# sarvex/redpanda

Measured on AMD Instinct MI355X. Metric: record-batch validate+parse(+decompress) GB/s per GPU and per 8-GPU node, higher is better.
Workload: dtype u8; 1 GPU; C2: 1,048,576 uncompressed Kafka v2 batches x 16,381 B (16 records x (16 B key + 995 B value)), 4096 partitions per GPU; Kafka CRC32C + internal header CRC + record walk + offset/timestamp index; batches_per_gpu=1048576, batches_total=1048576, partitions_total=4096, partitions_per_gpu=4096, parallelism=partition-shard x1

## Files before the change

### redpanda_amd/_build.py

```python
from __future__ import annotations

import os
import subprocess
from pathlib import Path

PKG = Path(__file__).resolve().parent
ROOT = PKG.parent
CSRC = PKG / "csrc"
INCLUDE = ROOT / "include"
CONDA = Path(os.environ.get("RPGPU_CODEC_PREFIX", "/opt/conda"))
ARCH = os.environ.get("PYTORCH_ROCM_ARCH", "gfx950")

LIBRPGPU = PKG / "librpgpu.so"
LIBRPGEN = PKG / "librpgen.so"

RPGPU_SRCS = ["rpgpu_kernels.hip", "rpgpu_decomp.hip", "rpgpu_sets.hip", "rpgpu_index.hip", "rpgpu_summary.hip", "rpgpu_compact.hip", "rpgpu_compact_rw.hip", "rpgpu_fetch.hip", "rpgpu_compress.hip", "rpgpu_stamp.hip", "rpgpu_legacy.hip", "rpgpu_pp.hip", "rpgpu_abi.cpp", "rpgpu_tables.cpp"]
RPGPU_HDRS = ["rpgpu_internal.h", "rpgpu_device.h", "rpgpu_walk.h", "rpgpu_copy.h", "rpgpu_legacy.h", "rpgpu_pp.h", "rpgpu_codec.h", "rpgpu_zstd.h", "rpgpu_zseq.h", "rpgpu_zblk.h", "rpgpu_wave.h", "rpgpu_inflate.h", "rpgpu_lz4c.h", "rpgpu_snappyc.h", "rpgpu_deflatec.h", "rpgpu_zstdc.h"]
RPGEN_SRCS = ["rpgen.cpp"]
RPGEN_HDRS = ["rpgen.h"]


def _stale(out: Path, srcs: list[Path]) -> bool:
    if not out.exists():
        return True
    t = out.stat().st_mtime
    return any(s.stat().st_mtime > t for s in srcs)


def _run(cmd: list[str]) -> None:
    r = subprocess.run(cmd, capture_output=True, text=True)
    if r.returncode != 0:
        raise RuntimeError(f"build failed: {' '.join(cmd)}\n{r.stdout}\n{r.stderr}")


def build_rpgpu(force: bool = False) -> Path:
    srcs = [CSRC / s for s in RPGPU_SRCS + RPGPU_HDRS] + [INCLUDE / "rpgpu.h"]
    if force or _stale(LIBRPGPU, srcs):
        from concurrent.futures import ThreadPoolExecutor

        obj = ROOT / "build" / "obj"
        obj.mkdir(parents=True, exist_ok=True)
        flags = [f"--offload-arch={ARCH}", "-O3", "-std=c++17", "-fPIC", f"-I{INCLUDE}", f"-I{CSRC}"]
        objs = [obj / (s + ".o") for s in RPGPU_SRCS]
        jobs = max(1, min(len(objs), os.cpu_count() or 1, 8))
        with ThreadPoolExecutor(jobs) as ex:
            list(ex.map(lambda so: _run(["hipcc", *flags, "-c", str(CSRC / so[0]), "-o", str(so[1])]),
                        zip(RPGPU_SRCS, objs)))
        tmp = LIBRPGPU.with_suffix(".so.tmp")
        _run(["hipcc", f"--offload-arch={ARCH}", "-shared", *[str(o) for o in objs], "-o", str(tmp)])
        os.replace(tmp, LIBRPGPU)
    return LIBRPGPU


def build_rpgen(force: bool = False) -> Path:
    srcs = [CSRC / s for s in RPGEN_SRCS + RPGEN_HDRS] + [INCLUDE / "rpgpu.h"]
    if force or _stale(LIBRPGEN, srcs):
        tmp = LIBRPGEN.with_suffix(".so.tmp")
        _run(["g++", "-O3", "-std=c++17", "-fPIC", "-shared", "-pthread",
              f"-I{INCLUDE}", f"-I{CSRC}", f"-I{CONDA / 'include'}",
              *[str(CSRC / s) for s in RPGEN_SRCS],
              f"-L{CONDA / 'lib'}", f"-Wl,-rpath,{CONDA / 'lib'}",
              "-llz4", "-lzstd", "-lsnappy", "-lz", "-o", str(tmp)])
        os.replace(tmp, LIBRPGEN)
    return LIBRPGEN


def build_all(force: bool = False) -> None:
    build_rpgpu(force)
    build_rpgen(force)


if __name__ == "__main__":
    build_all(force=True)
    print("built", LIBRPGPU, LIBRPGEN)
```

### redpanda_amd/csrc/rpgpu_kernels.hip

```cpp
#include "rpgpu_device.h"
#include "rpgpu_walk.h"

namespace rpgpu {

#ifdef RPGPU_DIAG_STAMPS
__device__ unsigned long long g_stamps[8];
struct Stamps {
    uint64_t st[8];
    uint64_t prev;
};
#define DIAG_PARAM , Stamps& sp
#define DIAG_PASS , sp
#define STAMP(i)                                          \
    do {                                                  \
        const uint64_t _t = __builtin_amdgcn_s_memtime(); \
        sp.st[i] += _t - sp.prev;                         \
        sp.prev = _t;                                     \
    } while (0)
#else
#define DIAG_PARAM
#define DIAG_PASS
#define STAMP(i) \
    do {         \
    } while (0)
#endif

struct Header {
    int32_t size_bytes;
    int64_t base_offset;
    int32_t type;
    int32_t crc;
    int16_t attrs;
    int32_t last_offset_delta;
    int64_t first_ts, max_ts, producer_id;
    int16_t producer_epoch;
    int32_t base_sequence, record_count;
};

struct Result {
    int32_t verdict;
    uint32_t crc, crc_expected, header_crc;
    Header h;
    uint32_t index_first, index_count;
};

__device__ __forceinline__ uint32_t u32s(uint32_t v) { return (uint32_t)__builtin_amdgcn_readfirstlane((int)v); }
__device__ __forceinline__ void write_result(rpgpu_batch_result* out, const Result& r) {
    if (lane_id() == 0) {
        const uint64_t bo = (uint64_t)r.h.base_offset, ft = (uint64_t)r.h.first_ts, mt = (uint64_t)r.h.max_ts;
        u32x4 a = {u32s((uint32_t)r.verdict), u32s(r.crc), u32s(r.crc_expected), u32s(r.header_crc)};
        u32x4 b = {u32s((uint32_t)r.h.size_bytes), u32s((uint32_t)r.h.record_count), u32s((uint32_t)bo),
                   u32s((uint32_t)(bo >> 32))};
        u32x4 c = {u32s((uint32_t)r.h.last_offset_delta),
                   u32s((uint32_t)(uint16_t)r.h.attrs | ((uint32_t)(r.h.attrs & 7) << 16) |
                        ((uint32_t)(uint8_t)r.h.type << 24)),
                   u32s((uint32_t)ft), u32s((uint32_t)(ft >> 32))};
        u32x4 d = {u32s((uint32_t)mt), u32s((uint32_t)(mt >> 32)), u32s(r.index_first), u32s(r.index_count)};
        u32x4* o = reinterpret_cast<u32x4*>(out);
        o[0] = a;
        o[1] = b;
        o[2] = c;
        o[3] = d;
    }
}

__device__ __forceinline__ void load_tables(uint32_t* s, const uint32_t* __restrict__ g) {
    for (int i = threadIdx.x; i < kTableWords / 4; i += blockDim.x)
        reinterpret_cast<u32x4*>(s)[i] = reinterpret_cast<const u32x4*>(g)[i];
    __syncthreads();
}

__device__ __forceinline__ uint32_t header_crc_vec(const uint32_t* sT, const Img64& D) {
    uint32_t win[16];
    win[0] = 0;
    win[1] = (D.w[1] << 24) ^ 0xff000000u;
    win[2] = ((D.w[1] >> 8) | (D.w[2] << 24)) ^ 0x00ffffffu;
#pragma unroll
    for (int m = 3; m < 16; m++) win[m] = (D.w[m - 1] >> 8) | (D.w[m] << 24);
    const uint32_t l = lane_id();
    uint32_t vwin = 0;
#pragma unroll
    for (int i = 0; i < 16; i++) vwin = writelane(vwin, win[i], i);
    const uint32_t w = __builtin_amdgcn_ds_bpermute((int)((l >> 2) << 2), vwin);
    const uint32_t byte = (w >> (8 * (l & 3))) & 255u;
    const uint32_t* hb = sT + kOffHB + l;
    uint32_t c = hb[(byte & 15u) * 64] ^ hb[(16u + (byte >> 4)) * 64];
    c ^= row_shl<1>(c);
    c ^= row_shl<2>(c);
    c ^= row_shl<4>(c);
    c ^= row_shl<8>(c);
    return ~(rdl(c, 0) ^ rdl(c, 16) ^ rdl(c, 32) ^ rdl(c, 48));
}

struct Geom {
    int32_t niter, g0;
};
__device__ __forceinline__ Geom geometry(int32_t n) {
    const int32_t niter = (n - 21 + 1023) >> 10;
    return Geom{niter, n - (niter << 10)};
}
__device__ __forceinline__ int32_t chunk_rows(int32_t niter) {
    return (niter + kRowsPerChunk - 1) & ~(kRowsPerChunk - 1);
}

struct Prefetch {
    u32x4 x[kRowsPerChunk];
    uint32_t hv;
    Geom gm;
};

typedef int32_t i32x4 __attribute__((ext_vector_type(4)));
__device__ __forceinline__ __amdgpu_buffer_rsrc_t batch_rsrc(const uint8_t* p) {
    return __builtin_amdgcn_make_buffer_rsrc(const_cast<uint8_t*>(p), 0, 0x7ffffff0, 0x00020000);
}
#ifndef RPGPU_ROW_AUX
#define RPGPU_ROW_AUX 2
#endif
__device__ __forceinline__ u32x4 load_row(__amdgpu_buffer_rsrc_t rs, const Geom& gm, int32_t row, uint32_t l) {
    const int32_t rb = row < gm.niter ? gm.g0 + (row << 10) : (int32_t)0x80000000;
    const i32x4 v = __builtin_amdgcn_raw_buffer_load_b128(rs, rb + (int32_t)(16 * l), 0, RPGPU_ROW_AUX);
    return (u32x4){(uint32_t)v.x, (uint32_t)v.y, (uint32_t)v.z, (uint32_t)v.w};
}

__device__ __forceinline__ void load_rows(u32x4 (&x)[kRowsPerChunk], __amdgpu_buffer_rsrc_t rs, const Geom& gm,
                                          int32_t cb, uint32_t l) {
#pragma unroll
    for (int k = 0; k < kRowsPerChunk; k++) x[k] = load_row(rs, gm, cb + k, l);
}

__device__ __forceinline__ Geom desc_geometry(const rpgpu_batch_desc& d) {
    return (d.length >= (uint32_t)kHeaderSize && !(d.flags & RPGPU_DESC_NULL_RECORDS)) ? geometry((int32_t)d.length)
                                                                                      : Geom{0, 0};
}

__device__ __forceinline__ u32x4 merge_header(u32x4 y, int32_t ro0, uint32_t v_img, uint32_t l) {
    if (ro0 >= kHeaderSize) return y;
    const int32_t ro = ro0 + 16 * (int32_t)l;
#pragma unroll
    for (int q = 0; q < 4; q++) {
        const int32_t o4 = ro + 4 * q;
        const uint32_t im = img_dword(v_img, o4);
        uint32_t keep;
        if (o4 >= kHeaderSize)
            keep = 0xffffffffu;
        else if (o4 + 4 <= kHeaderSize)
            keep = 0;
        else
            keep = 0xffffffffu << (8 * (uint32_t)(kHeaderSize - o4));
        const uint32_t raw = q == 0 ? y.x : q == 1 ? y.y : q == 2 ? y.z : y.w;
        const uint32_t v = (raw & keep) | (o4 >= kHeaderSize ? 0u : im);
        if (q == 0) y.x = v;
        if (q == 1) y.y = v;
        if (q == 2) y.z = v;
        if (q == 3) y.w = v;
    }
    return y;
}

__device__ __forceinline__ void process_batch(const uint32_t* __restrict__ sT, const rpgpu_batch_desc& d,
                                              uint32_t b, const uint8_t* __restrict__ data,
                                              rpgpu_batch_result* __restrict__ res, uint32_t index_first,
                                              Prefetch& pf, const rpgpu_batch_desc& nd,
                                              bool has_next DIAG_PARAM) {
    const uint32_t l = lane_id();
    const uint8_t* p = data + d.offset;
    const uint32_t len = d.length;
    Result r;
    r.verdict = RPGPU_V_OK;
    r.crc = r.crc_expected = r.header_crc = 0;
    r.h.size_bytes = r.h.type = r.h.crc = r.h.last_offset_delta = 0;
    r.h.base_sequence = r.h.record_count = 0;
    r.h.attrs = r.h.producer_epoch = 0;
    r.h.base_offset = r.h.first_ts = r.h.max_ts = r.h.producer_id = 0;
    r.index_first = index_first;
    r.index_count = 0;

    const uint32_t hv = pf.hv;
    Img64 H;
#pragma unroll
    for (int i = 0; i < 16; i++) H.w[i] = rdl(hv, i);
    Geom ngm{0, 0};
    const __amdgpu_buffer_rsrc_t nrs = batch_rsrc(data + (has_next ? nd.offset : 0));
    pf.hv = (uint32_t)__builtin_amdgcn_raw_buffer_load_b32(nrs, (int32_t)(4 * (l & 15)), 0, 0);
    if (has_next) ngm = desc_geometry(nd);

    Img64 D;
    D.clear();
    int64_t n;
    bool body_trunc = false;
    bool fail = false;
    if (d.flags & RPGPU_DESC_NULL_RECORDS) {
        n = 0;
        r.verdict = RPGPU_V_NULL_RECORDS;
        fail = true;
    } else if (d.format == RPGPU_FMT_KAFKA_WIRE) {
        const int32_t bl = (int32_t)H.get_be(8, 4);
        const uint64_t blen = (uint64_t)(int64_t)bl + 12u;
        if (blen <= (uint64_t)len) {
            n = (int64_t)blen;
        } else {
            n = len;
            body_trunc = true;
        }
        if (len < 12) {
            r.verdict = RPGPU_V_TOO_SMALL;
            fail = true;
        } else if (n < 17) {
            r.verdict = RPGPU_V_HDR_TRUNC_THROW;
            fail = true;
        } else if ((int8_t)H.byte(16) != 2) {
            r.verdict = RPGPU_V_BAD_MAGIC;
            fail = true;
        } else if (n < kHeaderSize) {
            r.verdict = RPGPU_V_HDR_TRUNC_THROW;
            fail = true;
        } else {
            r.h.size_bytes = (int32_t)((uint32_t)bl + 12u);
            r.h.base_offset = (int64_t)H.get_be(0, 8);
            r.h.type = 1;
            r.h.crc = (int32_t)H.get_be(17, 4);
            r.h.attrs = (int16_t)H.get_be(21, 2);
            r.h.last_offset_delta = (int32_t)H.get_be(23, 4);
            r.h.first_ts = (int64_t)H.get_be(27, 8);
            r.h.max_ts = (int64_t)H.get_be(35, 8);
            r.h.producer_id = (int64_t)H.get_be(43, 8);
            r.h.producer_epoch = (int16_t)H.get_be(51, 2);
            r.h.base_sequence = (int32_t)H.get_be(53, 4);
            r.h.record_count = (int32_t)H.get_be(57, 4);
            D.put_le(4, (uint32_t)r.h.size_bytes, 4);
            D.put_le(8, (uint64_t)r.h.base_offset, 8);
            D.put_le(16, 1, 1);
            D.put_le(17, (uint32_t)r.h.crc, 4);
            D.put_le(21, (uint16_t)r.h.attrs, 2);
            D.put_le(23, (uint32_t)r.h.last_offset_delta, 4);
            D.put_le(27, (uint64_t)r.h.first_ts, 8);
            D.put_le(35, (uint64_t)r.h.max_ts, 8);
            D.put_le(43, (uint64_t)r.h.producer_id, 8);
            D.put_le(51, (uint16_t)r.h.producer_epoch, 2);
            D.put_le(53, (uint32_t)r.h.base_sequence, 4);
            D.put_le(57, (uint32_t)r.h.record_count, 4);
        }
    } else {
        n = 0;
        if (len < kHeaderSize) {
            r.verdict = RPGPU_V_STREAM_SHORT;
            fail = true;
        } else {
            uint32_t any = 0;
#pragma unroll
            for (int i = 0; i < 15; i++) any |= H.w[i];
            any |= H.w[15] & 0xffu;
            if (any == 0) {
                r.verdict = RPGPU_V_FALLOCATED_ZERO;
                fail = true;
            } else {
#pragma unroll
                for (int i = 0; i < 16; i++) D.w[i] = H.w[i];
                D.w[15] &= 0xffu;
                r.h.size_bytes = (int32_t)H.get_le(4, 4);
                r.h.base_offset = (int64_t)H.get_le(8, 8);
                r.h.type = (int8_t)H.byte(16);
                r.h.crc = (int32_t)H.get_le(17, 4);
                r.h.attrs = (int16_t)H.get_le(21, 2);
                r.h.last_offset_delta = (int32_t)H.get_le(23, 4);
                r.h.first_ts = (int64_t)H.get_le(27, 8);
                r.h.max_ts = (int64_t)H.get_le(35, 8);
                r.h.producer_id = (int64_t)H.get_le(43, 8);
                r.h.producer_epoch = (int16_t)H.get_le(51, 2);
                r.h.base_sequence = (int32_t)H.get_le(53, 4);
                r.h.record_count = (int32_t)H.get_le(57, 4);
                n = (int64_t)r.h.size_bytes;
            }
        }
    }
    const bool is_disk = d.format != RPGPU_FMT_KAFKA_WIRE;
    const bool recrc = is_disk && (d.ops & RPGPU_OP_RECRC);
    if (!fail) {
        r.crc_expected = (uint32_t)r.h.crc;
        if (!recrc && ((d.ops & RPGPU_OP_HDRCRC) || is_disk)) r.header_crc = header_crc_vec(sT, D);
        if (is_disk) {
            if (!recrc && r.header_crc != H.w[0]) {
                r.verdict = RPGPU_V_HDR_CRC_MISMATCH;
                fail = true;
            } else if (r.h.size_bytes < kHeaderSize || (int64_t)r.h.size_bytes > (int64_t)len) {
                r.verdict = RPGPU_V_STREAM_SHORT;
                fail = true;
            }
        }
    }
    if (fail) {
        load_rows(pf.x, nrs, ngm, 0, l);
        pf.gm = ngm;
        write_result(res + b, r);
        return;
    }

    Img64 B;
    B.clear();
    B.put_be(21, (uint16_t)r.h.attrs, 2);
    B.put_be(23, (uint32_t)r.h.last_offset_delta, 4);
    B.put_be(27, (uint64_t)r.h.first_ts, 8);
    B.put_be(35, (uint64_t)r.h.max_ts, 8);
    B.put_be(43, (uint64_t)r.h.producer_id, 8);
    B.put_be(51, (uint16_t)r.h.producer_epoch, 2);
    B.put_be(53, (uint32_t)r.h.base_sequence, 4);
    B.put_be(57, (uint32_t)r.h.record_count, 4);
    B.w[5] ^= 0xffffff00u;
    B.w[6] ^= 0x000000ffu;
    uint32_t v_img = 0;
#pragma unroll
    for (int i = 0; i < 16; i++) v_img = (l == (uint32_t)i) ? B.w[i] : v_img;

    const Geom gm = geometry((int32_t)n);
    const int32_t nrows = chunk_rows(gm.niter);
    const bool pf_ok = pf.gm.niter == gm.niter && pf.gm.g0 == gm.g0;
    const uint32_t* sN = sT + kOffN;
    const __amdgpu_buffer_rsrc_t rs = batch_rsrc(p);
    const __amdgpu_buffer_rsrc_t nrs_rows = batch_rsrc(data + (has_next ? nd.offset : 0));
    uint32_t c = 0;
    STAMP(0);
    if (!pf_ok) load_rows(pf.x, rs, gm, 0, l);
    pf.x[0] = merge_header(pf.x[0], gm.g0, v_img, l);
    pf.x[1] = merge_header(pf.x[1], gm.g0 + 1024, v_img, l);
    for (int32_t cb = 0; cb < nrows; cb += kRowsPerChunk) {
        const bool last_chunk = cb + kRowsPerChunk >= nrows;
        const __amdgpu_buffer_rsrc_t lrs = last_chunk ? nrs_rows : rs;
        const Geom lg = last_chunk ? ngm : gm;
        const int32_t lrow = last_chunk ? 0 : cb + kRowsPerChunk;
#pragma unroll
        for (int k = 0; k < kRowsPerChunk; k++) {
            u32x4 y = pf.x[k];
            y.x ^= c;
            c = crc_block(sN, y);
            pf.x[k] = load_row(lrs, lg, lrow + k, l);
        }
    }
    pf.gm = ngm;
    STAMP(1);
#ifndef RPGPU_DIAG_NO_COMBINE
    c = combine64(sT + kOffW, c);
    if (nrows != gm.niter) c = apply8(sT + kOffU + (nrows - gm.niter) * 128, c);
#endif
    r.crc = ~rdl(c, 0);
#if defined(RPGPU_DIAG_NO_COMBINE) || defined(RPGPU_DIAG_NO_LOOKUP)
    asm volatile("" ::"v"(c));
    r.crc = r.crc_expected;
#endif
    if (recrc) {
        r.crc_expected = r.crc;
        r.h.crc = (int32_t)r.crc;
        D.put_le(17, r.crc, 4);
        r.header_crc = header_crc_vec(sT, D);
    }
    STAMP(2);

    const uint8_t codec = (uint8_t)(r.h.attrs & 7);
    if (r.crc != r.crc_expected) {
        r.verdict = RPGPU_V_CRC_MISMATCH;
    } else if (body_trunc) {
        r.verdict = RPGPU_V_BODY_TRUNC_THROW;
    } else if (codec > 4) {
        r.verdict = RPGPU_V_BAD_CODEC_THROW;
    }
    write_result(res + b, r);
    STAMP(3);
}

__global__ __launch_bounds__(kValidateThreads) void validate_kernel(
    const rpgpu_batch_desc* __restrict__ descs, uint32_t b0, uint32_t n, const uint8_t* __restrict__ data,
    rpgpu_batch_result* __restrict__ res, rpgpu_record_index* __restrict__ index,
    const uint32_t* __restrict__ local_first, const uint32_t* __restrict__ caps,
    const uint64_t* __restrict__ block_base, uint64_t index_cap, const uint32_t* __restrict__ tables) {
    __shared__ __attribute__((aligned(16))) uint32_t sT[kTableWords];
    load_tables(sT, tables);
    const uint32_t wave = threadIdx.x >> 6;
    const uint32_t gw = __builtin_amdgcn_readfirstlane(blockIdx.x * kWavesPerBlock + wave);
    const uint32_t nw = gridDim.x * kWavesPerBlock;
#ifdef RPGPU_DIAG_STAMPS
    Stamps sp{};
    sp.prev = __builtin_amdgcn_s_memtime();
#endif
    Prefetch pf;
    pf.gm = Geom{0, 0};
    if (b0 + gw < n) {
        const rpgpu_batch_desc d0 = sload_desc(descs + b0 + gw);
        const uint8_t* p0 = data + d0.offset;
        const __amdgpu_buffer_rsrc_t rs0 = batch_rsrc(p0);
        pf.hv = (uint32_t)__builtin_amdgcn_raw_buffer_load_b32(rs0, (int32_t)(4 * (lane_id() & 15)), 0, 0);
        pf.gm = desc_geometry(d0);
        load_rows(pf.x, rs0, pf.gm, 0, lane_id());
    }
    for (uint32_t b = b0 + gw; b < n; b += nw) {
        const rpgpu_batch_desc d = sload_desc(descs + b);
        const bool has_next = b + nw < n;
        const rpgpu_batch_desc nd = sload_desc(descs + (has_next ? b + nw : b));
        process_batch(sT, d, b, data, res, 0u, pf, nd, has_next DIAG_PASS);
        STAMP(5);
    }
#ifdef RPGPU_DIAG_STAMPS
    if (lane_id() == 0)
        for (int i = 0; i < 6; i++) atomicAdd(&g_stamps[i], (unsigned long long)sp.st[i]);
#endif
}

__global__ __launch_bounds__(256) void walk_kernel(const rpgpu_batch_desc* __restrict__ descs, uint32_t b0,
                                                   uint32_t n,
                                                   const uint8_t* __restrict__ data,
                                                   rpgpu_batch_result* __restrict__ res,
                                                   rpgpu_record_index* __restrict__ index,
                                                   const uint32_t* __restrict__ local_first,
                                                   const uint32_t* __restrict__ caps,
                                                   const uint64_t* __restrict__ block_base, uint64_t index_cap,
                                                   uint32_t* __restrict__ wave_list, uint32_t* __restrict__ wave_count) {
    const uint32_t b = b0 + blockIdx.x * blockDim.x + threadIdx.x;
    WalkJob J;
    J.flags = 0;
    J.body = 0;
    J.base_offset = J.first_ts = 0;
    J.n = J.first = J.cap = J.b = 0;
    J.rc = 0;
    uint32_t first_all = 0;
    if (b < n) {
        const rpgpu_batch_desc d = descs[b];
        const rpgpu_batch_result& r = res[b];
        const uint64_t first = block_base[b / kScanBlock] + local_first[b];
        first_all = (uint32_t)first;
        if ((d.ops & (RPGPU_OP_PARSE | RPGPU_OP_INDEX)) && r.verdict == RPGPU_V_OK && r.codec == 0) {
            uint64_t cap = caps[b];
            if (first >= index_cap) cap = 0;
            else if (first + cap > index_cap) cap = index_cap - first;
            J.body = d.offset + kHeaderSize;
            J.base_offset = r.base_offset;
            J.first_ts = r.first_timestamp;
            J.n = (uint32_t)r.size_bytes - kHeaderSize;
            J.rc = r.record_count;
            J.first = (uint32_t)first;
            J.cap = (uint32_t)cap;
            J.b = b;
            J.flags = kJobLive | ((d.ops & RPGPU_OP_INDEX) ? kJobIndex : 0u);
            if (J.rc > kWaveWalkMin) {
                wave_list[atomicAdd(wave_count, 1u)] = b;
                J.flags = 0;
            }
        }
    }
    walk_lanes(data, J, index, res);
    if (b < n && !(J.flags & kJobLive)) reinterpret_cast<uint32_t*>(res + b)[14] = first_all;
}

__global__ __launch_bounds__(256) void walk_wave_kernel(const rpgpu_batch_desc* __restrict__ descs,
                                                        const uint8_t* __restrict__ data,
                                                        rpgpu_batch_result* __restrict__ res,
                                                        rpgpu_record_index* __restrict__ index,
                                                        const uint32_t* __restrict__ local_first,
                                                        const uint32_t* __restrict__ caps,
                                                        const uint64_t* __restrict__ block_base, uint64_t index_cap,
                                                        const uint32_t* __restrict__ wave_list,
                                                        const uint32_t* __restrict__ wave_count,
                                                        uint32_t* __restrict__ head) {
    const uint32_t cnt = *wave_count;
    for (;;) {
        uint32_t k = 0;
        if (lane_id() == 0) k = atomicAdd(head, 1u);
        k = __builtin_amdgcn_readfirstlane(k);
        if (k >= cnt) break;
        const uint32_t b = wave_list[k];
        const rpgpu_batch_desc d = descs[b];
        const rpgpu_batch_result& r = res[b];
        const uint64_t first = block_base[b / kScanBlock] + local_first[b];
        uint64_t cap = caps[b];
        if (first >= index_cap) cap = 0;
        else if (first + cap > index_cap) cap = index_cap - first;
        WalkJob J;
        J.body = d.offset + kHeaderSize;
        J.base_offset = r.base_offset;
        J.first_ts = r.first_timestamp;
        J.n = (uint32_t)r.size_bytes - kHeaderSize;
        J.rc = r.record_count;
        J.first = (uint32_t)first;
        J.cap = (uint32_t)cap;
        J.b = b;
        J.flags = kJobLive | ((d.ops & RPGPU_OP_INDEX) ? kJobIndex : 0u);
        int32_t verdict;
        uint32_t count;
        wave_walk_batch(data, J, index, verdict, count);
        if (lane_id() == 0) {
            uint32_t* o = reinterpret_cast<uint32_t*>(res + b);
            o[0] = (uint32_t)verdict;
            o[15] = count;
        }
    }
}

__device__ __forceinline__ uint32_t index_cap(const rpgpu_batch_desc& d, const uint8_t* data) {
    if (!(d.ops & (RPGPU_OP_PARSE | RPGPU_OP_INDEX)) || (d.flags & RPGPU_DESC_NULL_RECORDS)) return 0;
    const uint8_t* p = data + d.offset;
    const uint64_t len = d.length;
    if (len < (uint64_t)kHeaderSize) return 0;
    uint64_t n;
    int32_t rc;
    uint32_t attrs;
    if (d.format == RPGPU_FMT_KAFKA_WIRE) {
        const int32_t bl = (int32_t)bswap32(ld4(p + 8));
        const uint64_t blen = (uint64_t)(int64_t)bl + 12u;
        if (blen > len) return 0;
        n = blen;
        if (n < (uint64_t)kHeaderSize || p[16] != 2) return 0;
        attrs = ((uint32_t)p[21] << 8) | p[22];
        rc = (int32_t)bswap32(ld4(p + 57));
    } else {
        const int32_t sz = (int32_t)ld4(p + 4);
        if (sz < kHeaderSize || (uint64_t)sz > len) return 0;
        n = (uint64_t)sz;
        attrs = ((uint32_t)p[22] << 8) | p[21];
        rc = (int32_t)ld4(p + 57);
    }
    if ((attrs & 7u) != 0 || rc <= 0) return 0;
    uint64_t cap = (n - kHeaderSize) / 2;
    if ((uint64_t)rc < cap) cap = (uint64_t)rc;
    return (uint32_t)cap;
}

__global__ __launch_bounds__(kScanBlock) void caps_kernel(const rpgpu_batch_desc* __restrict__ descs,
                                                          uint32_t n, const uint8_t* __restrict__ data,
                                                          uint32_t* __restrict__ caps,
                                                          uint32_t* __restrict__ local_first,
                                                          uint64_t* __restrict__ block_sum) {
    __shared__ uint32_t wsum[kScanBlock / 64];
    const uint32_t i = blockIdx.x * kScanBlock + threadIdx.x;
    uint32_t cap = 0;
    if (i < n) cap = index_cap(descs[i], data);
    const uint32_t l = lane_id();
    uint32_t x = cap;
#pragma unroll
    for (int s = 1; s < 64; s <<= 1) {
        uint32_t t = __shfl_up(x, s, 64);
        if (l >= (uint32_t)s) x += t;
    }
    const uint32_t wv = threadIdx.x >> 6;
    if (l == 63) wsum[wv] = x;
    __syncthreads();
    uint32_t wbase = 0;
    for (uint32_t k = 0; k < wv; k++) wbase += wsum[k];
    if (i < n) {
        caps[i] = cap;
        local_first[i] = wbase + x - cap;
    }
    if (threadIdx.x == kScanBlock - 1) {
        uint64_t tot = 0;
        for (uint32_t k = 0; k < kScanBlock / 64; k++) tot += wsum[k];
        block_sum[blockIdx.x] = tot;
    }
}

__global__ __launch_bounds__(1024) void block_scan_kernel(uint64_t* __restrict__ block_sum, uint32_t nb,
                                                          uint64_t* __restrict__ total_out) {
    __shared__ uint64_t part[1024];
    const uint32_t t = threadIdx.x;
    const uint32_t per = (nb + 1023) / 1024;
    const uint32_t lo = t * per, hi = (lo + per < nb) ? lo + per : nb;
    uint64_t s = 0;
    for (uint32_t k = lo; k < hi; k++) s += block_sum[k];
    part[t] = s;
    __syncthreads();
    for (uint32_t off = 1; off < 1024; off <<= 1) {
        uint64_t v = (t >= off) ? part[t - off] : 0;
        __syncthreads();
        part[t] += v;
        __syncthreads();
    }
    uint64_t run = part[t] - s;
    for (uint32_t k = lo; k < hi; k++) {
        const uint64_t v = block_sum[k];
        block_sum[k] = run;
        run += v;
    }
    if (t == 1023 && total_out) *total_out = part[1023];
}

__global__ __launch_bounds__(kValidateThreads) void crc_ranges_kernel(
    const uint8_t* __restrict__ data, const uint64_t* __restrict__ offs, const uint32_t* __restrict__ lens,
    const uint32_t* __restrict__ seeds, uint32_t n, uint32_t* __restrict__ out,
    const uint32_t* __restrict__ tables) {
    __shared__ __attribute__((aligned(16))) uint32_t sT[kTableWords];
    load_tables(sT, tables);
    const uint32_t l = lane_id();
    const uint32_t wave = threadIdx.x >> 6;
    const uint32_t gw = __builtin_amdgcn_readfirstlane(blockIdx.x * kWavesPerBlock + wave);
    const uint32_t nw = gridDim.x * kWavesPerBlock;
    for (uint32_t i = gw; i < n; i += nw) {
        const uint8_t* base = data + offs[i];
        const int64_t len = lens[i];
        const uint32_t init = ~(seeds ? seeds[i] : 0u);
        const uint32_t crc = crc_range_wave(sT, base, len, init, l);
        if (l == 0) out[i] = crc;
    }
}

__device__ __forceinline__ bool header_all_zero(const Img64& H) {
    uint32_t any = 0;
#pragma unroll
    for (int i = 0; i < 15; i++) any |= H.w[i];
    any |= H.w[15] & 0xffu;
    return any == 0;
}

__global__ __launch_bounds__(kValidateThreads) void segment_parse_kernel(
    const uint8_t* __restrict__ data, const rpgpu_segment_read* __restrict__ reads, uint32_t nreads,
    rpgpu_segment_parse_result* __restrict__ results, rpgpu_batch_desc* __restrict__ descs,
    const uint32_t* __restrict__ tables) {
    __shared__ __attribute__((aligned(16))) uint32_t sT[kTableWords];
    load_tables(sT, tables);
    const uint32_t l = lane_id();
    const uint32_t gw = __builtin_amdgcn_readfirstlane(blockIdx.x * kWavesPerBlock + (threadIdx.x >> 6));
    const uint32_t nw = gridDim.x * kWavesPerBlock;
    for (uint32_t s = gw; s < nreads; s += nw) {
        const rpgpu_segment_read rd = reads[s];
        const uint8_t* seg = data + rd.offset;
        const uint64_t len = rd.length;
        const bool reader = rd.mode == RPGPU_PARSE_READER;
        const uint64_t max_buffer = rd.max_buffer ? rd.max_buffer : 32u * 1024u;
        uint64_t pos = 0, bytes_consumed = 0, phys = 0, buffer = 0;
        int32_t err = RPGPU_V_OK;
        bool exception = false, stopped = false, over_budget = false;
        bool codec_throw = false;
        uint32_t accepted = 0, skipped = 0;
        int64_t start_offset = rd.start_offset, expected = rd.expected_next_batch;
        uint64_t cfg_bytes = rd.bytes_consumed;
        const __amdgpu_buffer_rsrc_t rs = batch_rsrc(seg);
        for (;;) {
            const uint64_t rem = len - pos;
            if (rem == 0) {
                err = RPGPU_V_END_OF_STREAM;
                break;
            }
            if (rem < (uint64_t)kHeaderSize) {
                err = RPGPU_V_STREAM_SHORT;
                break;
            }
            const uint32_t hv = (uint32_t)__builtin_amdgcn_raw_buffer_load_b32(rs, (int32_t)(pos + 4 * (l & 15)), 0, 0);
            Img64 H;
#pragma unroll
            for (int i = 0; i < 16; i++) H.w[i] = rdl(hv, i);
            if (header_all_zero(H)) {
                err = RPGPU_V_FALLOCATED_ZERO;
                break;
            }
            Img64 D;
#pragma unroll
            for (int i = 0; i < 16; i++) D.w[i] = H.w[i];
            D.w[15] &= 0xffu;
            if (header_crc_vec(sT, D) != H.w[0]) {
                err = RPGPU_V_HDR_CRC_MISMATCH;
                break;
            }
            const int32_t size_bytes = (int32_t)H.get_le(4, 4);
            const int64_t base_offset = (int64_t)H.get_le(8, 8);
            const int8_t type = (int8_t)H.byte(16);
            const int32_t lod = (int32_t)H.get_le(23, 4);
            const int64_t max_ts = (int64_t)H.get_le(35, 8);
            const int64_t last = base_offset + lod;
            const uint64_t sz = (uint64_t)(int64_t)size_bytes;
            int decision = 0;
            if (reader) {
                if (base_offset < expected) {
                    exception = true;
                    break;
                }
                if (base_offset > rd.max_offset) {
                    decision = 2;
                } else if ((rd.strict_max_bytes || cfg_bytes) && cfg_bytes + sz > rd.max_bytes) {
                    over_budget = true;
                    decision = 2;
                } else if (last < start_offset) {
                    decision = 1;
                } else if (rd.has_type_filter && rd.type_filter != type) {
                    start_offset = last + 1;
                    decision = 1;
                } else if (rd.has_first_timestamp && rd.first_timestamp > max_ts) {
                    start_offset = last + 1;
                    decision = 1;
                }
            }
            if (decision == 2) {
                stopped = true;
                break;
            }
            const uint64_t body = (uint64_t)((int64_t)size_bytes - kHeaderSize);
            const uint64_t avail = len - pos - kHeaderSize;
            if (decision == 1) {
                expected = last + 1;
                phys += sz;
                if (body > avail) {
                    err = RPGPU_V_STREAM_SHORT;
                    break;
                }
                pos += kHeaderSize + body;
                bytes_consumed += sz;
                skipped++;
// ... 378 lines not shown
```

Before: 4022 GB/s.

## Pack batch result into lane-distributed register and drop Header struct

Replaces the per-batch Result/Header structs, which held many 64-bit scalar fields, with a single VGPR whose lanes each carry one result word, built with writelane. The result is then stored by lanes 0-15 in parallel instead of by lane 0 with readfirstlane packing. The header CRC now reuses the lane-distributed header image, and recrc patches only two lanes. It also adds a min-blocks launch bound of 8. The goal is to cut register pressure and raise occupancy in the validate kernel, at the risk of spills under the tighter launch bound and of subtle byte-swapping errors in the header rewrite.

```diff
diff --git a/redpanda_amd/_build.py b/redpanda_amd/_build.py
--- a/redpanda_amd/_build.py
+++ b/redpanda_amd/_build.py
@@ -33,6 +33,10 @@
         raise RuntimeError(f"build failed: {' '.join(cmd)}\n{r.stdout}\n{r.stderr}")
 
 
+def rpgpu_flags() -> list[str]:
+    return [f"--offload-arch={ARCH}", "-O3", "-std=c++17", "-fPIC", f"-I{INCLUDE}", f"-I{CSRC}"]
+
+
 def build_rpgpu(force: bool = False) -> Path:
     srcs = [CSRC / s for s in RPGPU_SRCS + RPGPU_HDRS] + [INCLUDE / "rpgpu.h"]
     if force or _stale(LIBRPGPU, srcs):
@@ -40,7 +44,7 @@
 
         obj = ROOT / "build" / "obj"
         obj.mkdir(parents=True, exist_ok=True)
-        flags = [f"--offload-arch={ARCH}", "-O3", "-std=c++17", "-fPIC", f"-I{INCLUDE}", f"-I{CSRC}"]
+        flags = rpgpu_flags()
         objs = [obj / (s + ".o") for s in RPGPU_SRCS]
         jobs = max(1, min(len(objs), os.cpu_count() or 1, 8))
         with ThreadPoolExecutor(jobs) as ex:
diff --git a/redpanda_amd/csrc/rpgpu_kernels.hip b/redpanda_amd/csrc/rpgpu_kernels.hip
--- a/redpanda_amd/csrc/rpgpu_kernels.hip
+++ b/redpanda_amd/csrc/rpgpu_kernels.hip
@@ -25,43 +25,32 @@
     } while (0)
 #endif
 
-struct Header {
-    int32_t size_bytes;
-    int64_t base_offset;
-    int32_t type;
-    int32_t crc;
-    int16_t attrs;
-    int32_t last_offset_delta;
-    int64_t first_ts, max_ts, producer_id;
-    int16_t producer_epoch;
-    int32_t base_sequence, record_count;
+__device__ __forceinline__ uint32_t lanes16(const Img64& I) {
+    uint32_t v = 0;
+#pragma unroll
+    for (int i = 0; i < 16; i++) v = writelane(v, I.w[i], i);
+    return v;
+}
+
+enum : int {
+    kResVerdict = 0,
+    kResCrc = 1,
+    kResCrcExpected = 2,
+    kResHeaderCrc = 3,
+    kResSizeBytes = 4,
+    kResRecordCount = 5,
+    kResBaseOffset = 6,
+    kResLastOffsetDelta = 8,
+    kResAttrsCodecType = 9,
+    kResFirstTs = 10,
+    kResMaxTs = 12,
+    kResIndexFirst = 14,
+    kResIndexCount = 15,
 };
-
-struct Result {
-    int32_t verdict;
-    uint32_t crc, crc_expected, header_crc;
-    Header h;
-    uint32_t index_first, index_count;
-};
-
-__device__ __forceinline__ uint32_t u32s(uint32_t v) { return (uint32_t)__builtin_amdgcn_readfirstlane((int)v); }
-__device__ __forceinline__ void write_result(rpgpu_batch_result* out, const Result& r) {
-    if (lane_id() == 0) {
-        const uint64_t bo = (uint64_t)r.h.base_offset, ft = (uint64_t)r.h.first_ts, mt = (uint64_t)r.h.max_ts;
-        u32x4 a = {u32s((uint32_t)r.verdict), u32s(r.crc), u32s(r.crc_expected), u32s(r.header_crc)};
-        u32x4 b = {u32s((uint32_t)r.h.size_bytes), u32s((uint32_t)r.h.record_count), u32s((uint32_t)bo),
-                   u32s((uint32_t)(bo >> 32))};
-        u32x4 c = {u32s((uint32_t)r.h.last_offset_delta),
-                   u32s((uint32_t)(uint16_t)r.h.attrs | ((uint32_t)(r.h.attrs & 7) << 16) |
-                        ((uint32_t)(uint8_t)r.h.type << 24)),
-                   u32s((uint32_t)ft), u32s((uint32_t)(ft >> 32))};
-        u32x4 d = {u32s((uint32_t)mt), u32s((uint32_t)(mt >> 32)), u32s(r.index_first), u32s(r.index_count)};
-        u32x4* o = reinterpret_cast<u32x4*>(out);
-        o[0] = a;
-        o[1] = b;
-        o[2] = c;
-        o[3] = d;
-    }
+__device__ __forceinline__ void store_result(rpgpu_batch_result* out, uint32_t rv) {
+    static_assert(sizeof(rpgpu_batch_result) == 64, "result layout");
+    const uint32_t l = lane_id();
+    if (l < 16) reinterpret_cast<uint32_t*>(out)[l] = rv;
 }
 
 __device__ __forceinline__ void load_tables(uint32_t* s, const uint32_t* __restrict__ g) {
@@ -70,19 +59,12 @@
     __syncthreads();
 }
 
-__device__ __forceinline__ uint32_t header_crc_vec(const uint32_t* sT, const Img64& D) {
-    uint32_t win[16];
-    win[0] = 0;
-    win[1] = (D.w[1] << 24) ^ 0xff000000u;
-    win[2] = ((D.w[1] >> 8) | (D.w[2] << 24)) ^ 0x00ffffffu;
-#pragma unroll
-    for (int m = 3; m < 16; m++) win[m] = (D.w[m - 1] >> 8) | (D.w[m] << 24);
+__device__ __forceinline__ uint32_t header_crc_lanes(const uint32_t* sT, uint32_t dv) {
     const uint32_t l = lane_id();
-    uint32_t vwin = 0;
-#pragma unroll
-    for (int i = 0; i < 16; i++) vwin = writelane(vwin, win[i], i);
-    const uint32_t w = __builtin_amdgcn_ds_bpermute((int)((l >> 2) << 2), vwin);
-    const uint32_t byte = (w >> (8 * (l & 3))) & 255u;
+    const int32_t k = (int32_t)l - 3;
+    const uint32_t w = __builtin_amdgcn_ds_bpermute((k >> 2) << 2, dv);
+    uint32_t byte = (w >> (8 * (k & 3))) & 255u;
+    byte = l < 7 ? 0u : (l < 11 ? byte ^ 255u : byte);
     const uint32_t* hb = sT + kOffHB + l;
     uint32_t c = hb[(byte & 15u) * 64] ^ hb[(16u + (byte >> 4)) * 64];
     c ^= row_shl<1>(c);
@@ -90,6 +72,9 @@
     c ^= row_shl<4>(c);
     c ^= row_shl<8>(c);
     return ~(rdl(c, 0) ^ rdl(c, 16) ^ rdl(c, 32) ^ rdl(c, 48));
+}
+__device__ __forceinline__ uint32_t header_crc_vec(const uint32_t* sT, const Img64& D) {
+    return header_crc_lanes(sT, lanes16(D));
 }
 
 struct Geom {
@@ -159,21 +144,12 @@
 
 __device__ __forceinline__ void process_batch(const uint32_t* __restrict__ sT, const rpgpu_batch_desc& d,
                                               uint32_t b, const uint8_t* __restrict__ data,
-                                              rpgpu_batch_result* __restrict__ res, uint32_t index_first,
-                                              Prefetch& pf, const rpgpu_batch_desc& nd,
-                                              bool has_next DIAG_PARAM) {
+                                              rpgpu_batch_result* __restrict__ res, Prefetch& pf,
+                                              const rpgpu_batch_desc& nd, bool has_next DIAG_PARAM) {
     const uint32_t l = lane_id();
     const uint8_t* p = data + d.offset;
     const uint32_t len = d.length;
-    Result r;
-    r.verdict = RPGPU_V_OK;
-    r.crc = r.crc_expected = r.header_crc = 0;
-    r.h.size_bytes = r.h.type = r.h.crc = r.h.last_offset_delta = 0;
-    r.h.base_sequence = r.h.record_count = 0;
-    r.h.attrs = r.h.producer_epoch = 0;
-    r.h.base_offset = r.h.first_ts = r.h.max_ts = r.h.producer_id = 0;
-    r.index_first = index_first;
-    r.index_count = 0;
+    int32_t verdict = RPGPU_V_OK;
 
     const uint32_t hv = pf.hv;
     Img64 H;
@@ -191,7 +167,7 @@
     bool fail = false;
     if (d.flags & RPGPU_DESC_NULL_RECORDS) {
         n = 0;
-        r.verdict = RPGPU_V_NULL_RECORDS;
+        verdict = RPGPU_V_NULL_RECORDS;
         fail = true;
     } else if (d.format == RPGPU_FMT_KAFKA_WIRE) {
         const int32_t bl = (int32_t)H.get_be(8, 4);
@@ -203,47 +179,39 @@
             body_trunc = true;
         }
         if (len < 12) {
-            r.verdict = RPGPU_V_TOO_SMALL;
+            verdict = RPGPU_V_TOO_SMALL;
             fail = true;
         } else if (n < 17) {
-            r.verdict = RPGPU_V_HDR_TRUNC_THROW;
+            verdict = RPGPU_V_HDR_TRUNC_THROW;
             fail = true;
         } else if ((int8_t)H.byte(16) != 2) {
-            r.verdict = RPGPU_V_BAD_MAGIC;
+            verdict = RPGPU_V_BAD_MAGIC;
             fail = true;
         } else if (n < kHeaderSize) {
-            r.verdict = RPGPU_V_HDR_TRUNC_THROW;
+            verdict = RPGPU_V_HDR_TRUNC_THROW;
             fail = true;
         } else {
-            r.h.size_bytes = (int32_t)((uint32_t)bl + 12u);
-            r.h.base_offset = (int64_t)H.get_be(0, 8);
-            r.h.type = 1;
-            r.h.crc = (int32_t)H.get_be(17, 4);
-            r.h.attrs = (int16_t)H.get_be(21, 2);
-            r.h.last_offset_delta = (int32_t)H.get_be(23, 4);
-            r.h.first_ts = (int64_t)H.get_be(27, 8);
-            r.h.max_ts = (int64_t)H.get_be(35, 8);
-            r.h.producer_id = (int64_t)H.get_be(43, 8);
-            r.h.producer_epoch = (int16_t)H.get_be(51, 2);
-            r.h.base_sequence = (int32_t)H.get_be(53, 4);
-            r.h.record_count = (int32_t)H.get_be(57, 4);
-            D.put_le(4, (uint32_t)r.h.size_bytes, 4);
-            D.put_le(8, (uint64_t)r.h.base_offset, 8);
+            D.put_le(4, (uint32_t)bl + 12u, 4);
+            D.put_le(8, (uint32_t)H.get_be(4, 4), 4);
+            D.put_le(12, (uint32_t)H.get_be(0, 4), 4);
             D.put_le(16, 1, 1);
-            D.put_le(17, (uint32_t)r.h.crc, 4);
-            D.put_le(21, (uint16_t)r.h.attrs, 2);
-            D.put_le(23, (uint32_t)r.h.last_offset_delta, 4);
-            D.put_le(27, (uint64_t)r.h.first_ts, 8);
-            D.put_le(35, (uint64_t)r.h.max_ts, 8);
-            D.put_le(43, (uint64_t)r.h.producer_id, 8);
-            D.put_le(51, (uint16_t)r.h.producer_epoch, 2);
-            D.put_le(53, (uint32_t)r.h.base_sequence, 4);
-            D.put_le(57, (uint32_t)r.h.record_count, 4);
+            D.put_le(17, (uint32_t)H.get_be(17, 4), 4);
+            D.put_le(21, (uint32_t)H.get_be(21, 2), 2);
+            D.put_le(23, (uint32_t)H.get_be(23, 4), 4);
+            D.put_le(27, (uint32_t)H.get_be(31, 4), 4);
+            D.put_le(31, (uint32_t)H.get_be(27, 4), 4);
+            D.put_le(35, (uint32_t)H.get_be(39, 4), 4);
+            D.put_le(39, (uint32_t)H.get_be(35, 4), 4);
+            D.put_le(43, (uint32_t)H.get_be(47, 4), 4);
+            D.put_le(47, (uint32_t)H.get_be(43, 4), 4);
+            D.put_le(51, (uint32_t)H.get_be(51, 2), 2);
+            D.put_le(53, (uint32_t)H.get_be(53, 4), 4);
+            D.put_le(57, (uint32_t)H.get_be(57, 4), 4);
         }
     } else {
         n = 0;
         if (len < kHeaderSize) {
-            r.verdict = RPGPU_V_STREAM_SHORT;
+            verdict = RPGPU_V_STREAM_SHORT;
             fail = true;
         } else {
             uint32_t any = 0;
@@ -251,39 +219,45 @@
             for (int i = 0; i < 15; i++) any |= H.w[i];
             any |= H.w[15] & 0xffu;
             if (any == 0) {
-                r.verdict = RPGPU_V_FALLOCATED_ZERO;
+                verdict = RPGPU_V_FALLOCATED_ZERO;
                 fail = true;
             } else {
 #pragma unroll
                 for (int i = 0; i < 16; i++) D.w[i] = H.w[i];
                 D.w[15] &= 0xffu;
-                r.h.size_bytes = (int32_t)H.get_le(4, 4);
-                r.h.base_offset = (int64_t)H.get_le(8, 8);
-                r.h.type = (int8_t)H.byte(16);
-                r.h.crc = (int32_t)H.get_le(17, 4);
-                r.h.attrs = (int16_t)H.get_le(21, 2);
-                r.h.last_offset_delta = (int32_t)H.get_le(23, 4);
-                r.h.first_ts = (int64_t)H.get_le(27, 8);
-                r.h.max_ts = (int64_t)H.get_le(35, 8);
-                r.h.producer_id = (int64_t)H.get_le(43, 8);
-                r.h.producer_epoch = (int16_t)H.get_le(51, 2);
-                r.h.base_sequence = (int32_t)H.get_le(53, 4);
-                r.h.record_count = (int32_t)H.get_le(57, 4);
-                n = (int64_t)r.h.size_bytes;
+                n = (int64_t)(int32_t)D.w[1];
             }
         }
     }
     const bool is_disk = d.format != RPGPU_FMT_KAFKA_WIRE;
     const bool recrc = is_disk && (d.ops & RPGPU_OP_RECRC);
+    const int32_t size_bytes = (int32_t)D.w[1];
+    const uint32_t attrs = (uint32_t)D.get_le(21, 2);
+    uint32_t crc_expected = (uint32_t)D.get_le(17, 4);
+    uint32_t rv = 0;
+    rv = writelane(rv, (uint32_t)size_bytes, kResSizeBytes);
+    rv = writelane(rv, (uint32_t)D.get_le(57, 4), kResRecordCount);
+    rv = writelane(rv, D.w[2], kResBaseOffset);
+    rv = writelane(rv, D.w[3], kResBaseOffset + 1);
+    rv = writelane(rv, (uint32_t)D.get_le(23, 4), kResLastOffsetDelta);
+    rv = writelane(rv, attrs | ((attrs & 7u) << 16) | (D.byte(16) << 24), kResAttrsCodecType);
+    rv = writelane(rv, (uint32_t)D.get_le(27, 4), kResFirstTs);
+    rv = writelane(rv, (uint32_t)D.get_le(31, 4), kResFirstTs + 1);
+    rv = writelane(rv, (uint32_t)D.get_le(35, 4), kResMaxTs);
+    rv = writelane(rv, (uint32_t)D.get_le(39, 4), kResMaxTs + 1);
+    rv = writelane(rv, crc_expected, kResCrcExpected);
+    uint32_t dv = 0;
     if (!fail) {
-        r.crc_expected = (uint32_t)r.h.crc;
-        if (!recrc && ((d.ops & RPGPU_OP_HDRCRC) || is_disk)) r.header_crc = header_crc_vec(sT, D);
+        dv = lanes16(D);
+        uint32_t header_crc = 0;
+        if (!recrc && ((d.ops & RPGPU_OP_HDRCRC) || is_disk)) header_crc = header_crc_lanes(sT, dv);
+        rv = writelane(rv, header_crc, kResHeaderCrc);
         if (is_disk) {
-            if (!recrc && r.header_crc != H.w[0]) {
-                r.verdict = RPGPU_V_HDR_CRC_MISMATCH;
+            if (!recrc && header_crc != H.w[0]) {
+                verdict = RPGPU_V_HDR_CRC_MISMATCH;
                 fail = true;
-            } else if (r.h.size_bytes < kHeaderSize || (int64_t)r.h.size_bytes > (int64_t)len) {
-                r.verdict = RPGPU_V_STREAM_SHORT;
+            } else if (size_bytes < kHeaderSize || (int64_t)size_bytes > (int64_t)len) {
+                verdict = RPGPU_V_STREAM_SHORT;
                 fail = true;
             }
         }
@@ -291,25 +265,30 @@
     if (fail) {
         load_rows(pf.x, nrs, ngm, 0, l);
         pf.gm = ngm;
-        write_result(res + b, r);
+        rv = writelane(rv, (uint32_t)verdict, kResVerdict);
+        store_result(res + b, rv);
         return;
     }
 
-    Img64 B;
-    B.clear();
-    B.put_be(21, (uint16_t)r.h.attrs, 2);
-    B.put_be(23, (uint32_t)r.h.last_offset_delta, 4);
-    B.put_be(27, (uint64_t)r.h.first_ts, 8);
-    B.put_be(35, (uint64_t)r.h.max_ts, 8);
-    B.put_be(43, (uint64_t)r.h.producer_id, 8);
-    B.put_be(51, (uint16_t)r.h.producer_epoch, 2);
-    B.put_be(53, (uint32_t)r.h.base_sequence, 4);
-    B.put_be(57, (uint32_t)r.h.record_count, 4);
-    B.w[5] ^= 0xffffff00u;
-    B.w[6] ^= 0x000000ffu;
-    uint32_t v_img = 0;
-#pragma unroll
-    for (int i = 0; i < 16; i++) v_img = (l == (uint32_t)i) ? B.w[i] : v_img;
+    uint32_t v_img;
+    {
+        Img64 B;
+        B.clear();
+        B.put_be(21, attrs, 2);
+        B.put_be(23, (uint32_t)D.get_le(23, 4), 4);
+        B.put_be(27, (uint32_t)D.get_le(31, 4), 4);
+        B.put_be(31, (uint32_t)D.get_le(27, 4), 4);
+        B.put_be(35, (uint32_t)D.get_le(39, 4), 4);
+        B.put_be(39, (uint32_t)D.get_le(35, 4), 4);
+        B.put_be(43, (uint32_t)D.get_le(47, 4), 4);
+        B.put_be(47, (uint32_t)D.get_le(43, 4), 4);
+        B.put_be(51, (uint32_t)D.get_le(51, 2), 2);
+        B.put_be(53, (uint32_t)D.get_le(53, 4), 4);
+        B.put_be(57, (uint32_t)D.get_le(57, 4), 4);
+        B.w[5] ^= 0xffffff00u;
+        B.w[6] ^= 0x000000ffu;
+        v_img = lanes16(B);
+    }
 
     const Geom gm = geometry((int32_t)n);
     const int32_t nrows = chunk_rows(gm.niter);
@@ -341,32 +320,34 @@
     c = combine64(sT + kOffW, c);
     if (nrows != gm.niter) c = apply8(sT + kOffU + (nrows - gm.niter) * 128, c);
 #endif
-    r.crc = ~rdl(c, 0);
+    uint32_t crc = ~rdl(c, 0);
 #if defined(RPGPU_DIAG_NO_COMBINE) || defined(RPGPU_DIAG_NO_LOOKUP)
     asm volatile("" ::"v"(c));
-    r.crc = r.crc_expected;
+    crc = crc_expected;
 #endif
+    rv = writelane(rv, crc, kResCrc);
     if (recrc) {
-        r.crc_expected = r.crc;
-        r.h.crc = (int32_t)r.crc;
-        D.put_le(17, r.crc, 4);
-        r.header_crc = header_crc_vec(sT, D);
+        crc_expected = crc;
+        dv = writelane(dv, (rdl(dv, 4) & 0x000000ffu) | (crc << 8), 4);
+        dv = writelane(dv, (rdl(dv, 5) & 0xffffff00u) | (crc >> 24), 5);
+        rv = writelane(rv, crc_expected, kResCrcExpected);
+        rv = writelane(rv, header_crc_lanes(sT, dv), kResHeaderCrc);
     }
     STAMP(2);
 
-    const uint8_t codec = (uint8_t)(r.h.attrs & 7);
-    if (r.crc != r.crc_expected) {
-        r.verdict = RPGPU_V_CRC_MISMATCH;
+    if (crc != crc_expected) {
+        verdict = RPGPU_V_CRC_MISMATCH;
     } else if (body_trunc) {
-        r.verdict = RPGPU_V_BODY_TRUNC_THROW;
-    } else if (codec > 4) {
-        r.verdict = RPGPU_V_BAD_CODEC_THROW;
-    }
-    write_result(res + b, r);
+        verdict = RPGPU_V_BODY_TRUNC_THROW;
+    } else if ((attrs & 7u) > 4) {
+        verdict = RPGPU_V_BAD_CODEC_THROW;
+    }
+    rv = writelane(rv, (uint32_t)verdict, kResVerdict);
+    store_result(res + b, rv);
     STAMP(3);
 }
 
-__global__ __launch_bounds__(kValidateThreads) void validate_kernel(
+__global__ __launch_bounds__(kValidateThreads, 8) void validate_kernel(
     const rpgpu_batch_desc* __restrict__ descs, uint32_t b0, uint32_t n, const uint8_t* __restrict__ data,
     rpgpu_batch_result* __restrict__ res, rpgpu_record_index* __restrict__ index,
     const uint32_t* __restrict__ local_first, const uint32_t* __restrict__ caps,
@@ -394,7 +375,7 @@
         const rpgpu_batch_desc d = sload_desc(descs + b);
         const bool has_next = b + nw < n;
         const rpgpu_batch_desc nd = sload_desc(descs + (has_next ? b + nw : b));
-        process_batch(sT, d, b, data, res, 0u, pf, nd, has_next DIAG_PASS);
+        process_batch(sT, d, b, data, res, pf, nd, has_next DIAG_PASS);
         STAMP(5);
     }
 #ifdef RPGPU_DIAG_STAMPS
```

Result: faster. 4063 GB/s (median of 6 runs) (+1.0%).
